# troylee/nnet-asr

Measured on AMD Instinct MI355X. Metric: training frames/sec (whole node), 440→2048×4→senone MLP, 1/2/4/8 MI355X, higher is better.
Workload: dtype f32; 1 GPU; TNet SGD step, 440x2048x2048x2048x2048x4000 sigmoid MLP + softmax xent; bunch_per_gpu=1024, global_bunch=1024, frames_resident_per_gpu=65536, parallelism=dp1

## Files before the change

### nnet-asr_amd/csrc/kernels/gemm_f32.hip

```cpp
#include <float.h>

#include <cstdlib>
#include <array>
#include <cstring>
#include <initializer_list>
#include <map>
#include <mutex>
#include <unordered_map>
#include <type_traits>

#include "kcommon.h"
#include "rbm_stats.h"
#include "gather.h"

namespace tnetk {

enum { EPI_STORE = 0, EPI_BIAS = 1, EPI_BIAS_SIG = 2, EPI_DSIG = 3, EPI_SGD = 4, EPI_BIAS_NSIG = 5,
       EPI_BIAS_NEG = 6, EPI_RBM = 7,
       EPI_DSIG_CS = 8, EPI_SGD_B = 9,
       EPI_STORE_BG = 10,
       EPI_BIAS_SIG_BIN = 11 };
constexpr int kColsumSlabRows = 32;
constexpr int kMaxSplit = 8;
constexpr int epi_base(int e) {
// ... 1585 lines not shown
              const int cl = ecol(j) + e - bn;
              if constexpr (VM == 4) {
                *reinterpret_cast<f32x4*>(ts + cl * LDP + rl0) =
                    f32x4{acc[4 * aq][NE * j + e][r], acc[4 * aq + 1][NE * j + e][r], acc[4 * aq + 2][NE * j + e][r],
                          acc[4 * aq + 3][NE * j + e][r]};
              } else {
#pragma unroll
                for (int m = 0; m < VM; ++m) ts[cl * LDP + rl0 + m] = acc[VM * aq + m][NE * j + e][r];
              }
            }
        }
      __syncthreads();
      const __amdgpu_buffer_rsrc_t rs_t = tile_rsrc(p.Ct + (long)bn * p.ldct + bm);
      for (int u = threadIdx.x; u < BN * Q; u += NT) {
        const int cl = u / Q, q4 = u % Q, col = bn + cl, row0 = bm + 4 * q4;
        if (col >= N || row0 >= M) continue;
        const f32x4 v = *reinterpret_cast<const f32x4*>(ts + cl * LDP + 4 * q4);
        if (row0 + 3 < M) {
          st_wt(rs_t, (long)cl * p.ldct + 4 * q4, v);
        } else {
#pragma unroll
          for (int m = 0; m < 4; ++m)
            if (row0 + m < M) p.Ct[(long)col * p.ldct + row0 + m] = v[m];
        }
      }
    }
  }
  }
  if constexpr (EPI == EPI_BIAS_SIG_BIN) binarize_tile<BM, BN, NT>(p, bm, bn);
  TNET_STAMP(3);
  TNET_STAMP_RT(5);
}

template <int BM, int BN, int BK, int WM, int WN, int S, bool A_KC, bool B_KC, int EPI, int SPK = 0>
__global__ __launch_bounds__(WM * WN * 64)
__attribute__((amdgpu_waves_per_eu((WM * WN + 3) / 4, (WM * WN + 3) / 4)))
void gemm16_sk_kernel(const GemmP p, const int G) {
  __shared__ __attribute__((aligned(16))) float smem[gemm16_smem_floats<BM, BN, BK, S, EPI, true>()];
  const int T = ((p.M + BM - 1) / BM) * ((p.N + BN - 1) / BN), KT = p.K / BK;
  const long I = (long)T * KT;
  const int b = blockIdx.x, xcd = b & 7, q8 = G >> 3, r8 = G & 7;
  const int v = (xcd < r8 ? xcd * (q8 + 1) : r8 * (q8 + 1) + (xcd - r8) * q8) + (b >> 3);
  const long s = (long)v * I / G, e = (long)(v + 1) * I / G;
  for (long k0 = s; k0 < e;) {
    const int t = (int)(k0 / KT);
    const long tb = (long)t * KT, te = tb + KT, k1 = e < te ? e : te;
    if (k0 != s) __syncthreads();
    const int w0 = (int)(((tb + 1) * G - 1) / I), w1 = (int)((te * G - 1) / I);
    GemmP q = p;
    q.ksplit = w1 - w0 + 1;
    const long kk = (k0 - tb) * BK;
    q.A = p.A + (A_KC ? kk : kk * p.lda);
    q.B = p.B + (B_KC ? kk : kk * p.ldb);
    q.K = (int)((k1 - k0) * BK);
    gemm16_body<BM, BN, BK, WM, WN, S, SPK, A_KC, B_KC, kEpiStreamK + EPI, true>(q, smem, t);
    k0 = k1;
  }
}

template <int BM, int BN, bool A_KC, bool B_KC, int EPI, bool PX>
__global__ __launch_bounds__(256) __attribute__((amdgpu_waves_per_eu(1, 1)))
void gemm16_split2_kernel(const GemmP p) {
  __shared__ __attribute__((aligned(16))) float smem[gemm16_smem_floats<BM, BN, 64, 2, EPI, PX>()];
  const int nwg = gridDim.x, b = blockIdx.x, xcd = b & 7, q8 = nwg >> 3, r8 = nwg & 7;
  const int v = (xcd < r8 ? xcd * (q8 + 1) : r8 * (q8 + 1) + (xcd - r8) * q8) + (b >> 3);
  GemmP q = p;
  const long kk = (long)(v & 1) * (p.K / 2);
  q.A = p.A + (A_KC ? kk : kk * p.lda);
  q.B = p.B + (B_KC ? kk : kk * p.ldb);
  q.K = p.K / 2;
  q.ksplit = 2;
  gemm16_body<BM, BN, 64, 2, 2, 2, 0, A_KC, B_KC, kEpiStreamK + EPI, PX>(q, smem, v >> 1);
}

template <int BM, int BN, int BK, int WM, int WN, int S, int SP, bool A_KC, bool B_KC, int EPI_T, bool PX = false>
__global__ __launch_bounds__((WM * WN + (SP == 2)) * 64)
__attribute__((amdgpu_waves_per_eu((WM * WN + (SP == 2) + 3) / 4, (WM * WN + (SP == 2) + 3) / 4)))
void gemm16_kernel(const GemmP p_in) {
  __shared__ __attribute__((aligned(16))) float smem[gemm16_smem_floats<BM, BN, BK, S, EPI_T, PX>()];
  gemm16_body<BM, BN, BK, WM, WN, S, SP, A_KC, B_KC, EPI_T, PX>(p_in, smem, blockIdx.x);
}

template <int BMA, int BNA, bool AKA, bool BKA, int EPIA, bool PXA, int BMB, int BNB, bool AKB, bool BKB, int EPIB,
          bool PXB, int SPA = 0, int SPB = 0, int KTA = 64, int STA = 2>
__global__ __launch_bounds__(256) __attribute__((amdgpu_waves_per_eu(1, 1)))
void gemm16_pair_kernel(const GemmP pa, const GemmP pb, const int na) {
  constexpr int SA = gemm16_smem_floats<BMA, BNA, KTA, STA, EPIA, PXA>(), SB = gemm16_smem_floats<BMB, BNB, 64, 2, EPIB, PXB>();
  __shared__ __attribute__((aligned(16))) float smem[SA > SB ? SA : SB];
  if ((int)blockIdx.x < na) gemm16_body<BMA, BNA, KTA, 2, 2, STA, SPA, AKA, BKA, EPIA, PXA>(pa, smem, blockIdx.x);
  else gemm16_body<BMB, BNB, 64, 2, 2, 2, SPB, AKB, BKB, EPIB, PXB>(pb, smem, (int)blockIdx.x - na);
}

template <int BM, int BN, int BK, int WM, int WN, int S>
__global__ __launch_bounds__(WM * WN * 64) __attribute__((amdgpu_waves_per_eu(1, 1)))
void gemm16_upd_pair_kernel(const GemmP pa, const GemmP pb, const int na) {
  __shared__ __attribute__((aligned(16))) float smem[gemm16_smem_floats<BM, BN, BK, S, EPI_SGD_B, false>()];
  if ((int)blockIdx.x < na) gemm16_body<BM, BN, BK, WM, WN, S, 0, false, false, EPI_SGD_B, false>(pa, smem, blockIdx.x);
  else gemm16_body<BM, BN, BK, WM, WN, S, 0, false, false, EPI_SGD_B, false>(pb, smem, (int)blockIdx.x - na);
}

template <int BM, int BN, int BK, int WM, int WN, int S, int EPI = EPI_SGD_B>
__global__ __launch_bounds__(WM * WN * 64) __attribute__((amdgpu_waves_per_eu(1, 1)))
void gemm16_upd_gather_kernel(const GemmP pa, const GemmP pb, const int na, const int nb, const BunchGatherP g) {
  __shared__ __attribute__((aligned(16))) float smem[gemm16_smem_floats<BM, BN, BK, S, EPI, false>()];
  const int b = blockIdx.x;
  if (b < na) gemm16_body<BM, BN, BK, WM, WN, S, 0, false, false, EPI, false>(pa, smem, b);
  else if (b < na + nb) gemm16_body<BM, BN, BK, WM, WN, S, 0, false, false, EPI, false>(pb, smem, b - na);
  else bunch_gather_block(g, b - na - nb, (int)gridDim.x - na - nb);
}

template <bool BD>
__global__ __launch_bounds__(256) __attribute__((amdgpu_waves_per_eu(1, 1)))
void gemm16_upd_mixed_gather_kernel(const GemmP pa, const GemmP pb, const int na, const int nb, const BunchGatherP g) {
  constexpr int SA = gemm16_smem_floats<128, 128, 64, 2, EPI_SGD_B, true>();
  constexpr int SB = BD ? gemm16_smem_floats<64, 64, 64, 2, EPI_SGD_B, false>()
                        : gemm16_smem_floats<64, 64, 32, 4, EPI_SGD_B, false>();
  __shared__ __attribute__((aligned(16))) float smem[SA > SB ? SA : SB];
  const int b = blockIdx.x;
  if (b < na) {
    gemm16_body<128, 128, 64, 2, 2, 2, 5, false, false, EPI_SGD_B, true>(pa, smem, b);
  } else if (b < na + nb) {
    if constexpr (BD) gemm16_body<64, 64, 64, 2, 2, 2, 5, false, false, EPI_SGD_B, false>(pb, smem, b - na);
    else gemm16_body<64, 64, 32, 4, 1, 4, 0, false, false, EPI_SGD_B, false>(pb, smem, b - na);
  } else {
    bunch_gather_block(g, b - na - nb, (int)gridDim.x - na - nb);
  }
}

template <bool PX, int SP = 0, bool BKC = true>
__global__ __launch_bounds__(256) __attribute__((amdgpu_waves_per_eu(1, 1)))
void gemm16_bwd_slabs_kernel(const GemmP p, const int na, const float* __restrict__ Et, const TnetMatrixDim dEt,
                             float* __restrict__ cpt, const long ldcpt, const int slabs, const int ncb) {
  __shared__ __attribute__((aligned(16))) float smem[gemm16_smem_floats<64, 128, 64, 2, EPI_DSIG_CS, PX>()];
  const int b = blockIdx.x;
  if (b < na) {
    gemm16_body<64, 128, 64, 2, 2, 2, SP, true, BKC, EPI_DSIG_CS, PX>(p, smem, b);
  } else {
    const int c = b - na;
    colsum_partial_block<true>(Et, dEt, cpt, slabs, 0x7fffffff, ldcpt, c % ncb, c / ncb, smem);
  }
}

__global__ __launch_bounds__(256) __attribute__((amdgpu_waves_per_eu(1, 1)))
void gemm16_rbm_update_stats_kernel(const GemmP p, const int na, const float* __restrict__ Vs, TnetMatrixDim dV,
                                    const float* __restrict__ Hs, TnetMatrixDim dH, int B, int nvb,
                                    float* __restrict__ vb, float* __restrict__ cvb, float* __restrict__ hb,
                                    float* __restrict__ chb, float scale, float mmt, double* __restrict__ stats,
                                    int nhb, const BunchGatherP g, const int ng) {
  constexpr int SG = gemm16_smem_floats<64, 64, 32, 4, EPI_RBM, false>();
  __shared__ __attribute__((aligned(16))) float smem[SG > RS_SMEM_FLOATS ? SG : RS_SMEM_FLOATS];
  const int b = blockIdx.x;
  if (b < na) gemm16_body<64, 64, 32, 4, 1, 4, 0, false, false, EPI_RBM, false>(p, smem, b);
  else if (b < na + ng) bunch_gather_block(g, b - na, ng);
  else rbm_stats_block(b - na - ng, smem, Vs, dV, Hs, dH, B, nvb, vb, cvb, hb, chb, scale, mmt, stats, nhb);
}
// ... 197 lines not shown
  X(m128x256k32s3, 1, 128, 256, 32, 2, 2, 3, 0)         \
  X(m64x64k64s2, 1, 64, 64, 64, 2, 2, 2, 0)             \
  X(m64x64k32s4, 1, 64, 64, 32, 2, 2, 4, 0)             \
  X(m32x64k64s2, 1, 32, 64, 64, 2, 2, 2, 0)             \
  X(m64x64a4, 1, 64, 64, 64, 2, 2, 2, 5)

enum GemmCfg {
#define X(name, ...) CFG_##name,
  TNET_GEMM_CFGS(X)
#undef X
  CFG_COUNT
};
static const char* kCfgNames[CFG_COUNT] = {
#define X(name, ...) #name,
    TNET_GEMM_CFGS(X)
#undef X
};

static int g_cfg = -2;
static int g_group = -1;
static int g_split = -1;
static int g_early = 1;
static int g_pair = 1;
static int g_pre0 = 1;
static int g_reserve = 0, g_cus = 0;
static int g_direct = -1;
static int g_kc = -1;
static int g_wt = 1;
extern "C" int tnetk_top_rows_shape_ok(const float* X, long ldx, const float* W, long ldw, int M, int N, int K);
extern "C" int tnetk_top_rows_partials(const float* X, long ldx, const float* W, long ldw, int M, int N, int K,
                                       float* part, long ldpart, void* stream);
static int forced_cfg();
static bool upd64_direct(const GemmP& p);
constexpr int kTopSlices = 4;
static float* splitk_workspace(size_t bytes, hipStream_t st);
static bool top_split_ok(const GemmP& p) {
  static const bool on = !(getenv("TNET_TOP_SPLIT") && getenv("TNET_TOP_SPLIT")[0] == '0');
  return on && forced_cfg() < 0 && g_split <= 0 && tnetk_top_rows_shape_ok(p.A, p.lda, p.B, p.ldb, p.M, p.N, p.K);
}
static float* top_split_partials(const GemmP& p, hipStream_t st, int* ldp_out) {
  const int ldp = 16 * ((p.N + 15) / 16);
  float* ws = splitk_workspace(sizeof(float) * kTopSlices * (size_t)p.M * ldp, st);
  if (!ws) return nullptr;
  if (tnetk_top_rows_partials(p.A, p.lda, p.B, p.ldb, p.M, p.N, p.K, ws, ldp, st) != TNET_OK) return nullptr;
  *ldp_out = ldp;
  return ws;
}
struct WeightShadow {
  float* t;
  long ld;
  int rows, cols;
  int kept;
};
static std::mutex g_shadow_mu;
static std::unordered_map<const float*, WeightShadow> g_shadow;
static thread_local int g_shadow_dropped = 0;
static void shadow_attach(GemmP& p) {
  p.Ct = nullptr;
  p.ldct = 0;
  g_shadow_dropped = 0;
  std::lock_guard<std::mutex> g(g_shadow_mu);
  auto it = g_shadow.find(p.C);
  if (it != g_shadow.end() && it->second.rows == p.M && it->second.cols == p.N) {
    p.Ct = it->second.t;
    p.ldct = it->second.ld;
  }
// ... 293 lines not shown
  int ks = 1;
  if (splittable) {
    int tbm, tbn, kind;
    cfg_shape(cfg, &tbm, &tbn, &kind);
    const long tiles = (long)cdiv(p.M, tbm) * cdiv(p.N, tbn);
    if (g_split > 0) {
      ks = g_split < kMaxSplit ? g_split : kMaxSplit;
    } else if (tiles < 100 && p.K >= 1024) {
      while (ks < kMaxSplit && tiles * ks * 2 <= 288) ks *= 2;
      const long t32 = (long)cdiv(p.M, 32) * cdiv(p.N, 64);
      if (cfg == CFG_m64x64k32s4w41 && ks >= 4 && t32 * (ks / 2) <= 288) {
        cfg = CFG_m32x64k64s2;
        kind = 1;
        ks /= 2;
      }
    }
    while (ks > 1 && (p.K % (4 * ks) != 0 || p.K / ks < 64)) ks /= 2;
    if (ks > 1 && kind != 1) cfg = CFG_m64x64k32s4w41;
  }
  return GemmPlan{cfg, ks};
}

template <bool A_KC, bool B_KC, int EPI>
static int launch_gemm(const GemmP& p_in, hipStream_t st) {
  if constexpr (EPI == EPI_DSIG_CS) {
    if constexpr (B_KC) return launch_colsum_bwd(p_in, st);
    else return launch_colsum_bwd_t(p_in, st);
  } else {
  if (p_in.M <= 0 || p_in.N <= 0) return TNET_OK;
  static const int noload = getenv("TNET_GEMM_DIAG") ? atoi(getenv("TNET_GEMM_DIAG")) : 0;
  GemmP p = p_in;
  p.diag_noload = noload;
  p.group = g_group > 0 ? g_group : 8;
  if (launch_split2<A_KC, B_KC, EPI>(p, st)) {
    TNET_LAUNCH_CHECK();
    return TNET_OK;
  }
  const GemmPlan pl = plan_gemm<A_KC>(p, epi_splittable(EPI));
  const int cfg = pl.cfg;
  if (pl.ks > 1) return launch_splitk<A_KC, B_KC, EPI>(p, cfg, pl.ks, st);
  bool sk_done = false;
  if (cfg == CFG_m64x128k64s2) sk_done = launch_sk<64, 128, A_KC, B_KC, EPI>(p, st);
  else if (cfg == CFG_m128x128k64s2) sk_done = launch_sk<128, 128, A_KC, B_KC, EPI>(p, st);
  if (sk_done) {
    TNET_LAUNCH_CHECK();
    return TNET_OK;
  }
  int rcfg = cfg;
  if (g_direct > 0 && forced_cfg() < 0 && !B_KC) {
    if (cfg == CFG_m64x128k64s2)
      rcfg = (g_direct == 3 || p.K <= 512) ? CFG_m64x128a4 : CFG_m64x128a8;
    else if (cfg == CFG_m128x128k64s2) rcfg = CFG_m128x128a4;
    else if (cfg == CFG_m128x256k32s3 && g_direct == 4) rcfg = CFG_m128x256a2;
  }
  if (g_kc >= 2 && forced_cfg() < 0 && A_KC && B_KC && cfg == CFG_m64x128k64s2) rcfg = CFG_m64x128c8;
  if constexpr (!A_KC && !B_KC && (EPI == EPI_SGD_B || EPI == EPI_SGD))
    if (forced_cfg() < 0 && cfg == CFG_m64x64k32s4w41 && upd64_direct(p)) rcfg = CFG_m64x64a4;
  bool ok = false;
  switch (rcfg) {
#define X(name, KIND, BM, BN, BK, WM, WN, S, IL) \
  case CFG_##name: ok = launch_cfg<KIND, BM, BN, BK, WM, WN, S, IL, A_KC, B_KC, EPI>(p, st); break;
    TNET_GEMM_CFGS(X)
#undef X
    default: return TNET_ERR_ARG;
  }
  if (!ok) launch_cfg<0, 64, 64, 32, 2, 2, 4, 0, A_KC, B_KC, EPI>(p, st);
// ... 84 lines not shown
static int launch_pair_upd_bwd(GemmP pu, GemmP pb, hipStream_t st) { return launch_pair_a_bwd<EPI_SGD_B>(pu, pb, st); }

static int cu_count() {
  if (!g_cus) {
    int dev = 0;
    hipDeviceProp_t prop;
    if (hipGetDevice(&dev) != hipSuccess || hipGetDeviceProperties(&prop, dev) != hipSuccess) return 0;
    g_cus = prop.multiProcessorCount;
  }
  return g_cus;
}
static bool split2_on() {
  if (g_split2 < 0) g_split2 = getenv("TNET_GEMM_SPLIT2") ? atoi(getenv("TNET_GEMM_SPLIT2")) : 0;
  return g_split2 != 0;
}

static int launch_upd_pair(GemmP pa, GemmP pb, hipStream_t st) {
  if (forced_cfg() >= 0 || !g_pair) return TNET_ERR_UNSUPPORTED;
  if (pa.M <= 0 || pa.N <= 0 || pb.M <= 0 || pb.N <= 0) return TNET_ERR_UNSUPPORTED;
  if (!g_cus) {
    int dev = 0;
    hipDeviceProp_t prop;
    if (hipGetDevice(&dev) != hipSuccess || hipGetDeviceProperties(&prop, dev) != hipSuccess)
      return TNET_ERR_UNSUPPORTED;
    g_cus = prop.multiProcessorCount;
  }
  const int na = cdiv(pa.M, 64) * cdiv(pa.N, 64), nb = cdiv(pb.M, 64) * cdiv(pb.N, 64);
  if (na + nb > g_cus - g_reserve) return TNET_ERR_UNSUPPORTED;
  for (const GemmP* q : {&pa, &pb})
    if (4 * (32L * q->lda + q->M) >= (1L << 32) || 4 * (32L * q->ldb + q->N) >= (1L << 32)) return TNET_ERR_UNSUPPORTED;
  pa.group = pb.group = g_group > 0 ? g_group : 8;
  pa.early_issue = pb.early_issue = g_early;
  pa.wt = pb.wt = g_wt;
  gemm16_upd_pair_kernel<64, 64, 32, 4, 1, 4><<<na + nb, 256, 0, st>>>(pa, pb, na);
  TNET_LAUNCH_CHECK();
  return TNET_OK;
}

static bool aligned16(const void* q) { return ((uintptr_t)q & 15) == 0; }

static int check_common(const GemmP& p) {
  if (p.M < 0 || p.N < 0 || p.K < 0) return TNET_ERR_ARG;
  if ((p.lda & 3) || (p.ldb & 3) || (p.ldc & 3)) return TNET_ERR_ARG;
  if (!aligned16(p.A) || !aligned16(p.B) || !aligned16(p.C)) return TNET_ERR_ARG;
  return TNET_OK;
}

}

using namespace tnetk;

extern "C" int tnet_sgemm(char transa, char transb, int m, int n, int k, float alpha, const float* A, int lda,
                          const float* B, int ldb, float beta, float* C, int ldc, void* stream) {
  GemmP p{};
  p.M = m; p.N = n; p.K = k;
  p.A = A; p.lda = lda; p.B = B; p.ldb = ldb; p.C = C; p.ldc = ldc;
  p.alpha = alpha; p.beta = beta;
  int st = check_common(p);
  if (st) return st;
  const bool ta = (transa == 'T' || transa == 't'), tb = (transb == 'T' || transb == 't');
  hipStream_t s = (hipStream_t)stream;
  if (k == 0) {
    if (beta == 1.f) return TNET_OK;
    TnetMatrixDim d{m, n, ldc};
    return tnetF_add_scaled(0.f, C, ldc, beta, C, d, stream);
  }
  if (!ta && !tb) return launch_gemm<true, false, EPI_STORE>(p, s);
// ... 437 lines not shown

extern "C" int tnet_affine_update_bias_pair(const float* X, TnetMatrixDim dX, const float* E, TnetMatrixDim dE,
                                           float* W, TnetMatrixDim dW, float* corrW, int strideCorr, float scale,
                                           float mmt, float l2, const float* colpart, int ldcolpart, float* b,
                                           float* corr_b, const float* X2, TnetMatrixDim dX2, const float* E2,
                                           TnetMatrixDim dE2, float* W2, TnetMatrixDim dW2, float* corrW2,
                                           int strideCorr2, float scale2, float mmt2, float l22,
                                           const float* colpart2, int ldcolpart2, float* b2, float* corr_b2,
                                           void* stream) {
  GemmP pa, pb;
  int st = update_bias_params(pa, X, dX, E, dE, W, dW, corrW, strideCorr, scale, mmt, l2, colpart, ldcolpart, b,
                              corr_b);
  if (st) return st;
  st = update_bias_params(pb, X2, dX2, E2, dE2, W2, dW2, corrW2, strideCorr2, scale2, mmt2, l22, colpart2, ldcolpart2,
                          b2, corr_b2);
  if (st) return st;
  if (W == W2 || b == b2 || (corrW && corrW == corrW2)) return TNET_ERR_ARG;
  shadow_attach(pb);
  shadow_attach(pa);
  const int rc = launch_upd_pair(pa, pb, (hipStream_t)stream);
  shadow_done(pa, rc);
  return shadow_done(pb, rc);
}

namespace tnetk {
static bool upd64_direct(const GemmP& p) {
  static const bool on = !(getenv("TNET_UPD64_DIRECT") && getenv("TNET_UPD64_DIRECT")[0] == '0');
  auto a16p = [](const void* v) { return ((uintptr_t)v & 15) == 0; };
  return on && g_direct > 0 && p.ksplit <= 1 && (long)cdiv(p.M, 64) * cdiv(p.N, 64) >= 200 && p.K / 64 >= 1 &&
         p.M % 4 == 0 && p.N % 4 == 0 && !(p.lda & 3) && !(p.ldb & 3) && a16p(p.A) && a16p(p.B) &&
         4 * ((long)p.K * p.lda) < (1L << 31) && 4 * ((long)p.K * p.ldb) < (1L << 31);
}

static bool upd_mixed_ok(const GemmP& pa, const GemmP& pb) {
  static const bool on = !(getenv("TNET_UPD_MIXED") && getenv("TNET_UPD_MIXED")[0] == '0');
  if (!on || !g_pair || g_reserve > 0 || g_direct <= 0 || forced_cfg() >= 0) return false;
  const GemmPlan la = plan_gemm<false>(pa, true), lb = plan_gemm<false>(pb, true);
  if (la.cfg != CFG_m128x128k64s2 || la.ks != 1 || lb.cfg != CFG_m64x64k32s4w41 || lb.ks != 1) return false;
  auto a16p = [](const void* v) { return ((uintptr_t)v & 15) == 0; };
  const bool dir = pa.K / 64 >= 1 && !(pa.lda & 3) && !(pa.ldb & 3) && a16p(pa.A) && a16p(pa.B) && pa.M % 4 == 0 &&
                   pa.N % 4 == 0 && 4 * ((long)pa.K * pa.lda) < (1L << 31) && 4 * ((long)pa.K * pa.ldb) < (1L << 31);
  if (!dir || !px_exact<128, 128, EPI_SGD_B>(pa)) return false;
  if (4 * (64L * pa.lda + pa.M) >= (1L << 32) || 4 * (64L * pa.ldb + pa.N) >= (1L << 32)) return false;
  if (4 * (32L * pb.lda + pb.M) >= (1L << 32) || 4 * (32L * pb.ldb + pb.N) >= (1L << 32)) return false;
  return true;
}
}

extern "C" int tnet_affine_update_bias_gather(const float* X, TnetMatrixDim dX, const float* E, TnetMatrixDim dE,
                                              float* W, TnetMatrixDim dW, float* corrW, int strideCorr, float scale,
                                              float mmt, float l2, const float* colpart, int ldcolpart, float* b,
                                              float* corr_b, const float* X2, TnetMatrixDim dX2, const float* E2,
                                              TnetMatrixDim dE2, float* W2, TnetMatrixDim dW2, float* corrW2,
                                              int strideCorr2, float scale2, float mmt2, float l22,
                                              const float* colpart2, int ldcolpart2, float* b2, float* corr_b2,
                                              float* y, const float* x, int* labels_out, const int* labels_in,
                                              const int* copy_from, TnetMatrixDim dy, TnetMatrixDim dx,
                                              void* stream) {
  GemmP pa, pb{};
  int st = update_bias_params(pa, X, dX, E, dE, W, dW, corrW, strideCorr, scale, mmt, l2, colpart, ldcolpart, b,
                              corr_b);
  if (st) return st;
  const bool two = X2 != nullptr;
  if (two) {
    st = update_bias_params(pb, X2, dX2, E2, dE2, W2, dW2, corrW2, strideCorr2, scale2, mmt2, l22, colpart2,
                            ldcolpart2, b2, corr_b2);
// ... 11 lines not shown
    return std::array<ByteSpan, 4>{span_of(q.C, q.M, q.ldc, 4), span_of(q.corr, q.M, q.ldcorr, 4),
                                   span_of(q.bvec, q.N, 1, 4), span_of(q.bcorr, q.N, 1, 4)};
  };
  shadow_attach(pa);
  if (two) shadow_attach(pb);
  const ByteSpan cta = span_of(pa.Ct, pa.N, pa.ldct, 4), ctb = span_of(two ? pb.Ct : nullptr, pb.N, pb.ldct, 4);
  const auto ra = reads(pa), rb = reads(pb);
  const auto wa = writes(pa), wb = writes(pb);
  if (!gather_independent(y, x, labels_out, labels_in, copy_from, dy, dx, {ra[0], ra[1], ra[2], rb[0], rb[1], rb[2]},
                          {wa[0], wa[1], wa[2], wa[3], wb[0], wb[1], wb[2], wb[3], cta, ctb}))
    return TNET_ERR_ARG;
  if (any_overlap({cta, ctb}, {ra[0], ra[1], ra[2], rb[0], rb[1], rb[2], wa[0], wa[1], wa[2], wa[3], wb[0], wb[1],
                               wb[2], wb[3]}) ||
      spans_overlap(cta, ctb))
    return TNET_ERR_ARG;
  const int c4 = (dy.cols + 3) & ~3;
  if (((uintptr_t)y & 15) || ((uintptr_t)x & 15) || (dy.stride & 3) || (dx.stride & 3) || c4 > dy.stride ||
      c4 > dx.stride)
    return TNET_ERR_UNSUPPORTED;
  if (forced_cfg() >= 0 || split2_on() || g_split > 0) return TNET_ERR_UNSUPPORTED;
  if (pa.M <= 0 || pa.N <= 0 || (two && (pb.M <= 0 || pb.N <= 0))) return TNET_ERR_UNSUPPORTED;
  int na, nb = 0;
  if (two && upd_mixed_ok(pa, pb)) {
    na = cdiv(pa.M, 128) * cdiv(pa.N, 128);
    nb = cdiv(pb.M, 64) * cdiv(pb.N, 64);
    const int cus = cu_count();
    if (cus <= 0) return TNET_ERR_UNSUPPORTED;
    const int spare = cus - nb;
    const int ng = spare < 8 ? 8 : spare > 64 ? 64 : spare;
    pa.group = pb.group = g_group > 0 ? g_group : 8;
    pa.early_issue = pb.early_issue = g_early;
    pa.wt = pb.wt = g_wt;
    BunchGatherP g{y, x, labels_out, labels_in, copy_from, dy.rows, c4, dy.stride, dx.stride};
    if (upd64_direct(pb)) gemm16_upd_mixed_gather_kernel<true><<<na + nb + ng, 256, 0, (hipStream_t)stream>>>(pa, pb, na, nb, g);
    else gemm16_upd_mixed_gather_kernel<false><<<na + nb + ng, 256, 0, (hipStream_t)stream>>>(pa, pb, na, nb, g);
    TNET_LAUNCH_CHECK();
    shadow_done(pa, TNET_OK);
    return shadow_done(pb, TNET_OK);
  }
  if (two) {
    if (!g_pair) return TNET_ERR_UNSUPPORTED;
    na = cdiv(pa.M, 64) * cdiv(pa.N, 64);
    nb = cdiv(pb.M, 64) * cdiv(pb.N, 64);
  } else {
    const GemmPlan pl = plan_gemm<false>(pa, epi_splittable(EPI_SGD_B));
    if (pl.cfg != CFG_m64x64k32s4w41 || pl.ks != 1) return TNET_ERR_UNSUPPORTED;
    na = cdiv(pa.M, 64) * cdiv(pa.N, 64);
  }
  for (const GemmP* q : {&pa, &pb}) {
    if (q == &pb && !two) break;
    if (4 * (32L * q->lda + q->M) >= (1L << 32) || 4 * (32L * q->ldb + q->N) >= (1L << 32)) return TNET_ERR_UNSUPPORTED;
  }
  const int cus = cu_count();
  if (cus <= 0) return TNET_ERR_UNSUPPORTED;
  const int spare = cus - g_reserve - na - nb;
  if (two && na + nb > cus - g_reserve) return TNET_ERR_UNSUPPORTED;
  if (spare < 8) return TNET_ERR_UNSUPPORTED;
  const int ng = spare < 64 ? spare : 64;
  pa.group = pb.group = g_group > 0 ? g_group : 8;
  pa.early_issue = pb.early_issue = g_early;
  pa.wt = pb.wt = g_wt;
  BunchGatherP g{y, x, labels_out, labels_in, copy_from, dy.rows, c4, dy.stride, dx.stride};
  gemm16_upd_gather_kernel<64, 64, 32, 4, 1, 4><<<na + nb + ng, 256, 0, (hipStream_t)stream>>>(pa, pb, na, nb, g);
  TNET_LAUNCH_CHECK();
  shadow_done(pa, TNET_OK);
  if (two) shadow_done(pb, TNET_OK);
  return TNET_OK;
}

static int update_bwd_pair(const float* X, TnetMatrixDim dX, const float* E, TnetMatrixDim dE, float* W,
                           TnetMatrixDim dW, float* corrW, int strideCorr, float scale, float mmt, float l2,
                           const float* colpart, int ldcolpart, float* b, float* corr_b, const float* E2,
                           TnetMatrixDim dE2, const float* W2, TnetMatrixDim dW2, const float* Ybelow, int strideYbelow,
                           float* Eo, TnetMatrixDim dEo, float* colpart2, int ldcolpart2, void* stream, bool bwd_t) {
  if (dX.rows != dE.rows || dW.rows != dX.cols || dW.cols != dE.cols || !colpart || !b || ldcolpart < dE.cols)
    return TNET_ERR_ARG;
  if (mmt != 0.f && (!corrW || !corr_b)) return TNET_ERR_ARG;
  const int w2_k = bwd_t ? dW2.rows : dW2.cols, w2_n = bwd_t ? dW2.cols : dW2.rows;
  if (dE2.cols != w2_k || dEo.rows != dE2.rows || dEo.cols != w2_n || !Ybelow || !colpart2 ||
      ldcolpart2 < dEo.cols || !aligned16(Ybelow) || (strideYbelow & 3))
    return TNET_ERR_ARG;
  if (W == W2) return TNET_ERR_ARG;
  GemmP pu{};
  pu.M = dX.cols; pu.N = dE.cols; pu.K = dX.rows;
  pu.A = X; pu.lda = dX.stride; pu.B = E; pu.ldb = dE.stride; pu.C = W; pu.ldc = dW.stride;
  pu.corr = (mmt != 0.f || corrW) ? corrW : nullptr; pu.ldcorr = strideCorr;
  if (pu.corr && (pu.ldcorr & 3)) return TNET_ERR_ARG;
  pu.scale = scale; pu.mmt = mmt; pu.l2 = l2;
  pu.bpart = colpart; pu.ldbpart = ldcolpart; pu.bslabs = tnet_colsum_slabs(dE.rows);
  pu.bvec = b; pu.bcorr = mmt != 0.f ? corr_b : nullptr; pu.bscale = scale; pu.bmmt = mmt;
  int st = check_common(pu);
  if (st) return st;
  GemmP pb{};
  pb.M = dE2.rows; pb.N = w2_n; pb.K = dE2.cols;
  pb.A = E2; pb.lda = dE2.stride; pb.B = W2; pb.ldb = dW2.stride; pb.C = Eo; pb.ldc = dEo.stride;
  pb.alpha = 1.f; pb.beta = 0.f;
// ... 136 lines not shown
                          {wa[0], wa[1], wb[0], wb[1]}))
    return TNET_ERR_ARG;
  const int c4 = (dy.cols + 3) & ~3;
  if (((uintptr_t)y & 15) || ((uintptr_t)x & 15) || (dy.stride & 3) || (dx.stride & 3) || c4 > dy.stride ||
      c4 > dx.stride)
    return TNET_ERR_UNSUPPORTED;
  if (forced_cfg() >= 0 || split2_on() || g_split > 0) return TNET_ERR_UNSUPPORTED;
  if (pa.M <= 0 || pa.N <= 0 || (two && (pb.M <= 0 || pb.N <= 0))) return TNET_ERR_UNSUPPORTED;
  int na, nb = 0;
  if (two) {
    if (!g_pair) return TNET_ERR_UNSUPPORTED;
    na = cdiv(pa.M, 64) * cdiv(pa.N, 64);
    nb = cdiv(pb.M, 64) * cdiv(pb.N, 64);
  } else {
    const GemmPlan pl = plan_gemm<false>(pa, epi_splittable(EPI_STORE_BG));
    if (pl.cfg != CFG_m64x64k32s4w41 || pl.ks != 1) return TNET_ERR_UNSUPPORTED;
    na = cdiv(pa.M, 64) * cdiv(pa.N, 64);
  }
  for (const GemmP* q : {&pa, &pb}) {
    if (q == &pb && !two) break;
    if (4 * (32L * q->lda + q->M) >= (1L << 32) || 4 * (32L * q->ldb + q->N) >= (1L << 32)) return TNET_ERR_UNSUPPORTED;
  }
  const int cus = cu_count();
  if (cus <= 0) return TNET_ERR_UNSUPPORTED;
  if (two && na + nb > cus - g_reserve) return TNET_ERR_UNSUPPORTED;
  const int spare = cus - g_reserve - na - nb;
  if (spare < 8) return TNET_ERR_UNSUPPORTED;
  const int ng = spare < 64 ? spare : 64;
  pa.group = pb.group = g_group > 0 ? g_group : 8;
  pa.early_issue = pb.early_issue = g_early;
  pa.wt = pb.wt = g_wt;
  BunchGatherP g{y, x, labels_out, labels_in, copy_from, dy.rows, c4, dy.stride, dx.stride};
  gemm16_upd_gather_kernel<64, 64, 32, 4, 1, 4, EPI_STORE_BG><<<na + nb + ng, 256, 0, (hipStream_t)stream>>>(
      pa, pb, na, nb, g);
  TNET_LAUNCH_CHECK();
  return TNET_OK;
}

extern "C" int tnet_affine_grad(const float* X, TnetMatrixDim dX, const float* E, TnetMatrixDim dE, float* G,
                                TnetMatrixDim dG, void* stream) {
  if (dX.rows != dE.rows || dG.rows != dX.cols || dG.cols != dE.cols) return TNET_ERR_ARG;
  GemmP p{};
  p.M = dX.cols; p.N = dE.cols; p.K = dX.rows;
  p.A = X; p.lda = dX.stride; p.B = E; p.ldb = dE.stride; p.C = G; p.ldc = dG.stride;
  p.alpha = 1.f; p.beta = 0.f;
  int st = check_common(p);
  if (st) return st;
  return launch_gemm<false, false, EPI_STORE>(p, (hipStream_t)stream);
}

extern "C" int tnet_gemm_config(const char* name) {
  forced_cfg();
  char base[64] = "auto";
  int split = -1, rsv = -1, s2 = -1;
  if (name) {
    const char* plus = strchr(name, '+');
    const size_t n = plus ? (size_t)(plus - name) : strlen(name);
    if (n >= sizeof(base)) return TNET_ERR_ARG;
    memcpy(base, name, n);
    base[n] = 0;
    while (plus) {
      if (!strncmp(plus, "+sk", 3) && atoi(plus + 3) >= 1) split = atoi(plus + 3);
      else if (!strncmp(plus, "+rsv", 4) && plus[4] >= '0' && plus[4] <= '9') rsv = atoi(plus + 4);
      else if (!strncmp(plus, "+s2", 3) && (plus[3] == '0' || plus[3] == '1')) s2 = plus[3] - '0';
      else return TNET_ERR_ARG;
      plus = strchr(plus + 1, '+');
    }
  }
  int cfg = -2;
  if (!strcmp(base, "auto")) cfg = -1;
  for (int i = 0; i < CFG_COUNT; i++)
    if (!strcmp(base, kCfgNames[i])) cfg = i;
  if (cfg == -2) return TNET_ERR_ARG;
  g_cfg = cfg;
  g_split = split;
  if (rsv >= 0) g_reserve = rsv;
  if (s2 >= 0) g_split2 = s2;
  return TNET_OK;
}

extern "C" int tnet_gemm_reserve(int cus) {
  if (cus < 0) return TNET_ERR_ARG;
  forced_cfg();
  g_reserve = cus;
  return TNET_OK;
}

#ifdef TNET_GEMM_STAMP
extern "C" int tnet_diag_stamps(unsigned long long* host, int n_wg) {
  if (n_wg > 8192) n_wg = 8192;
  return hipMemcpyFromSymbol(host, HIP_SYMBOL(g_tnet_stamps), sizeof(unsigned long long) * 6 * n_wg, 0,
                             hipMemcpyDeviceToHost) == hipSuccess ? TNET_OK : TNET_ERR_LAUNCH;
}
extern "C" int tnet_diag_stamps_clear() {
  void* a = nullptr;
  if (hipGetSymbolAddress(&a, HIP_SYMBOL(g_tnet_stamps)) != hipSuccess) return TNET_ERR_RUNTIME;
  return hipMemset(a, 0, sizeof(g_tnet_stamps)) == hipSuccess && hipDeviceSynchronize() == hipSuccess
             ? TNET_OK : TNET_ERR_RUNTIME;
}
#endif
```

Measured before the change: 1.019 million frames/s.

## Add intra-block K-split 64x64 weight-update kernel with register-ring buffer loads

Adds a new 64x64 SGD weight-update GEMM body in which each of the four waves takes a quarter of the K range. Each wave streams its operands directly from global memory into a register ring using buffer loads interleaved with MFMAs, and the partial tiles are reduced through LDS before the fused SGD/momentum/bias epilogue. It is dispatched automatically wherever the planner would pick the 64x64 direct-update config, including the pair, gather and mixed-gather launchers. The aim is to avoid LDS staging and the per-K-step barriers on the tall-K update GEMMs. In exchange it uses a large register footprint and adds a cross-wave reduction step.

```diff
diff --git a/nnet-asr_amd/csrc/kernels/gemm_f32.hip b/nnet-asr_amd/csrc/kernels/gemm_f32.hip
--- a/nnet-asr_amd/csrc/kernels/gemm_f32.hip
+++ b/nnet-asr_amd/csrc/kernels/gemm_f32.hip
@@ -1641,6 +1641,212 @@
   TNET_STAMP_RT(5);
 }
 
+constexpr int kKsplitSmemFloats = 3 * 64 * 64;
+template <int EPI>
+__device__ __forceinline__ void upd64_ksplit_body(const GemmP& p, float* __restrict__ smem, const int bid_x) {
+  static_assert(EPI == EPI_SGD || EPI == EPI_SGD_B, "SGD epilogues only");
+  constexpr int BM = 64, BN = 64, DD = 4, NR = 8;
+  TNET_STAMP_RT(4);
+  TNET_STAMP(0);
+  const int M = p.M, N = p.N, K = p.K;
+  const int nbn = (N + BN - 1) / BN, nbm = (M + BM - 1) / BM;
+  const int nwg = nbm * nbn;
+  const int bid = bid_x, xcd = bid & 7, q8 = nwg >> 3, r8 = nwg & 7;
+  const int L = (xcd < r8 ? xcd * (q8 + 1) : r8 * (q8 + 1) + (xcd - r8) * q8) + (bid >> 3);
+  const int grp = p.group, per_group = grp * nbn;
+  const int first_m = (L / per_group) * grp;
+  const int gsz = min(nbm - first_m, grp);
+  const int bm = (first_m + (L % per_group) % gsz) * BM, bn = ((L % per_group) / gsz) * BN;
+
+  const int lane = threadIdx.x & 63, wid = __builtin_amdgcn_readfirstlane(threadIdx.x >> 6);
+  const int lg = lane >> 4, li = lane & 15;
+  const int KQ = 16 * ((((K + 3) >> 2) + 15) >> 4);
+  const int k0 = wid * KQ, k1 = min(K, k0 + KQ);
+  const int nch = (k1 - k0) >> 4, rem = (k1 - k0) & 15;
+
+  const int ca = max(min(bm + 4 * li, M - 4), 0), cb = max(min(bn + 4 * li, N - 4), 0);
+  unsigned oA[4], oB[4];
+#pragma unroll
+  for (int s = 0; s < 4; ++s) {
+    oA[s] = 4u * (unsigned)((4 * lg + s) * p.lda + ca);
+    oB[s] = 4u * (unsigned)((4 * lg + s) * p.ldb + cb);
+  }
+  const int cA = 64 * p.lda, cB = 64 * p.ldb;
+  const unsigned long long ba = (unsigned long long)(uintptr_t)(p.A + (long)k0 * p.lda),
+                           bb = (unsigned long long)(uintptr_t)(p.B + (long)k0 * p.ldb);
+  const u32x4 dA = {(unsigned)ba, (unsigned)(ba >> 32), 0x7FFFFFF0u, 0x00020000u};
+  const u32x4 dB = {(unsigned)bb, (unsigned)(bb >> 32), 0x7FFFFFF0u, 0x00020000u};
+
+  f32x4 acc[4][4];
+#pragma unroll
+  for (int a = 0; a < 4; ++a)
+#pragma unroll
+    for (int b = 0; b < 4; ++b) acc[a][b] = f32x4{0.f, 0.f, 0.f, 0.f};
+
+  f32x4 ring[DD][NR];
+  auto ld = [&](int c, int r) {
+    f32x4 v;
+    if (r < 4) asm volatile("buffer_load_dwordx4 %0, %1, %2, %3 offen" : "=v"(v) : "v"(oA[r]), "s"(dA), "s"(c * cA));
+    else asm volatile("buffer_load_dwordx4 %0, %1, %2, %3 offen" : "=v"(v) : "v"(oB[r - 4]), "s"(dB), "s"(c * cB));
+    return v;
+  };
+  constexpr int WV = (DD - 2) * NR;
+  auto wait_slot = [&](f32x4 (&q)[NR]) {
+    asm volatile("s_waitcnt vmcnt(%8)"
+                 : "+v"(q[0]), "+v"(q[1]), "+v"(q[2]), "+v"(q[3]), "+v"(q[4]), "+v"(q[5]), "+v"(q[6]), "+v"(q[7])
+                 : "n"(WV));
+  };
+#pragma unroll
+  for (int j = 0; j < DD - 1; ++j)
+#pragma unroll
+    for (int r = 0; r < NR; ++r) ring[j][r] = ld(min(j, nch - 1), r);
+  asm volatile("" ::: "memory");
+
+  const int erow0 = bm + 16 * lg + 4 * wid, ecol = bn + 4 * li;
+  const bool has_q = p.corr != nullptr;
+  f32x4 pre_w[4], pre_q[4];
+#pragma unroll
+  for (int a = 0; a < 4; ++a) {
+    pre_w[a] = pre_q[a] = f32x4{0.f, 0.f, 0.f, 0.f};
+    if (erow0 + a < M && ecol < N) {
+      pre_w[a] = *reinterpret_cast<const f32x4*>(p.C + (long)(erow0 + a) * p.ldc + ecol);
+      if (has_q) pre_q[a] = *reinterpret_cast<const f32x4*>(p.corr + (long)(erow0 + a) * p.ldcorr + ecol);
+    }
+  }
+  BiasPre bpre;
+  if constexpr (EPI == EPI_SGD_B)
+    if (bm == 0) bias_pre_load<BN, false>(p, bn, bpre);
+  TNET_STAMP(1);
+
+  auto chunk_mfmas = [&](const f32x4 (&q)[NR], auto&& filler) {
+    int mi = 0;
+#pragma unroll
+    for (int s2 = 0; s2 < 4; ++s2)
+#pragma unroll
+      for (int a = 0; a < 4; ++a)
+#pragma unroll
+        for (int b = 0; b < 4; ++b) {
+          acc[a][b] = __builtin_amdgcn_mfma_f32_16x16x4f32(q[s2][a], q[4 + s2][b], acc[a][b], 0, 0, 0);
+          filler(mi);
+          ++mi;
+        }
+  };
+  for (int c0 = 0; c0 < nch; c0 += DD) {
+#pragma unroll
+    for (int j = 0; j < DD; ++j) {
+      if (c0 + j >= nch) break;
+      const int cn = min(c0 + j + DD - 1, nch - 1);
+      __builtin_amdgcn_sched_barrier(0);
+      wait_slot(ring[j]);
+      __builtin_amdgcn_sched_barrier(0);
+      chunk_mfmas(ring[j], [&](int mi) {
+        if (mi < NR) {
+          __builtin_amdgcn_sched_barrier(0);
+          ring[(j + DD - 1) % DD][mi] = ld(cn, mi);
+          __builtin_amdgcn_sched_barrier(0);
+        }
+      });
+    }
+  }
+  asm volatile("s_waitcnt vmcnt(0)" ::: "memory");
+  if (rem) {
+    f32x4 t[NR];
+#pragma unroll
+    for (int s = 0; s < 4; ++s) {
+      const int k = k0 + 16 * nch + 4 * lg + s, kk = min(k, K - 1);
+      const f32x4 x = *reinterpret_cast<const f32x4*>(p.A + (long)kk * p.lda + ca);
+      const f32x4 e = *reinterpret_cast<const f32x4*>(p.B + (long)kk * p.ldb + cb);
+      const f32x4 z = {0.f, 0.f, 0.f, 0.f};
+      t[s] = k < k1 ? x : z;
+      t[4 + s] = k < k1 ? e : z;
+    }
+    chunk_mfmas(t, [](int) {});
+  }
+  TNET_STAMP(2);
+
+  auto vec = [&](int a, int r) { return f32x4{acc[a][0][r], acc[a][1][r], acc[a][2][r], acc[a][3][r]}; };
+  f32x4 own[4];
+#pragma unroll
+  for (int r = 0; r < 4; ++r) {
+    if (wid == r) {
+#pragma unroll
+      for (int a = 0; a < 4; ++a) own[a] = vec(a, r);
+    } else {
+      const int sl = wid < r ? wid : wid - 1;
+#pragma unroll
+      for (int a = 0; a < 4; ++a)
+        *reinterpret_cast<f32x4*>(smem + ((4 * r + a) * 3 + sl) * 256 + 4 * lane) = vec(a, r);
+    }
+  }
+  __syncthreads();
+  const __amdgpu_buffer_rsrc_t rs_c = tile_rsrc(p.C + (long)bm * p.ldc + bn);
+  const __amdgpu_buffer_rsrc_t rs_q = tile_rsrc(p.corr ? p.corr + (long)bm * p.ldcorr + bn : p.C);
+  f32x4 part[4][3];
+#pragma unroll
+  for (int a = 0; a < 4; ++a)
+#pragma unroll
+    for (int sl = 0; sl < 3; ++sl)
+      part[a][sl] = *reinterpret_cast<const f32x4*>(smem + ((4 * wid + a) * 3 + sl) * 256 + 4 * lane);
+  f32x4 upd[4];
+#pragma unroll
+  for (int a = 0; a < 4; ++a) upd[a] = f32x4{0.f, 0.f, 0.f, 0.f};
+#pragma unroll
+  for (int a = 0; a < 4; ++a) {
+    const int row = erow0 + a;
+    if (row >= M || ecol >= N) continue;
+    const f32x4 p0 = wid == 0 ? own[a] : part[a][0];
+    const f32x4 p1 = wid == 0 ? part[a][0] : wid == 1 ? own[a] : part[a][1];
+    const f32x4 p2 = wid <= 1 ? part[a][1] : wid == 2 ? own[a] : part[a][2];
+    const f32x4 p3 = wid == 3 ? own[a] : part[a][2];
+    const f32x4 v = ((p0 + p1) + p2) + p3;
+    f32x4 o, qn;
+#pragma unroll
+    for (int e = 0; e < 4; ++e) {
+      const float c = has_q ? v[e] + p.mmt * pre_q[a][e] : v[e];
+      qn[e] = c;
+      float w = pre_w[a][e];
+      w = w + p.scale * c;
+      w = w + p.l2 * w;
+      o[e] = w;
+    }
+    upd[a] = o;
+    if (p.wt) {
+      st_wt(rs_c, (long)(row - bm) * p.ldc + (ecol - bn), o);
+      if (has_q) st_wt(rs_q, (long)(row - bm) * p.ldcorr + (ecol - bn), qn);
+    } else {
+      *reinterpret_cast<f32x4*>(p.C + (long)row * p.ldc + ecol) = o;
+      if (has_q) *reinterpret_cast<f32x4*>(p.corr + (long)row * p.ldcorr + ecol) = qn;
+    }
+  }
+  if (p.Ct) {
+    constexpr int LDP = BM + 4, Q = BM / 4;
+    static_assert(BN * LDP <= kKsplitSmemFloats, "shadow image fits the partial tiles' LDS");
+    __syncthreads();
+#pragma unroll
+    for (int e = 0; e < 4; ++e)
+      *reinterpret_cast<f32x4*>(smem + (4 * li + e) * LDP + 16 * lg + 4 * wid) =
+          f32x4{upd[0][e], upd[1][e], upd[2][e], upd[3][e]};
+    __syncthreads();
+    const __amdgpu_buffer_rsrc_t rs_t = tile_rsrc(p.Ct + (long)bn * p.ldct + bm);
+    for (int u = threadIdx.x; u < BN * Q; u += 256) {
+      const int cl = u / Q, q4 = u % Q;
+      if (bn + cl >= N || bm + 4 * q4 >= M) continue;
+      st_wt(rs_t, (long)cl * p.ldct + 4 * q4, *reinterpret_cast<const f32x4*>(smem + cl * LDP + 4 * q4));
+    }
+  }
+  if constexpr (EPI == EPI_SGD_B)
+    if (bm == 0) bias_pre_finish<BN, false>(p, bn, bpre);
+  TNET_STAMP(3);
+  TNET_STAMP_RT(5);
+}
+
+template <int EPI>
+__global__ __launch_bounds__(256) __attribute__((amdgpu_waves_per_eu(1, 1)))
+void gemm16_upd_ksplit_kernel(const GemmP p) {
+  __shared__ __attribute__((aligned(16))) float smem[kKsplitSmemFloats];
+  upd64_ksplit_body<EPI>(p, smem, blockIdx.x);
+}
+
 template <int BM, int BN, int BK, int WM, int WN, int S, bool A_KC, bool B_KC, int EPI, int SPK = 0>
 __global__ __launch_bounds__(WM * WN * 64)
 __attribute__((amdgpu_waves_per_eu((WM * WN + 3) / 4, (WM * WN + 3) / 4)))
@@ -1700,36 +1906,55 @@
   else gemm16_body<BMB, BNB, 64, 2, 2, 2, SPB, AKB, BKB, EPIB, PXB>(pb, smem, (int)blockIdx.x - na);
 }
 
-template <int BM, int BN, int BK, int WM, int WN, int S>
+template <int BM, int BN, int BK, int WM, int WN, int S, bool KS = false>
 __global__ __launch_bounds__(WM * WN * 64) __attribute__((amdgpu_waves_per_eu(1, 1)))
-void gemm16_upd_pair_kernel(const GemmP pa, const GemmP pb, const int na) {
+void gemm16_upd_pair_kernel(const GemmP pa, const GemmP pb, const int na, const int ksa, const int ksb) {
+  static_assert(!KS || (BM == 64 && BN == 64 && WM * WN == 4 && S * (BM + BN) * BK >= kKsplitSmemFloats), "ksplit tile");
   __shared__ __attribute__((aligned(16))) float smem[gemm16_smem_floats<BM, BN, BK, S, EPI_SGD_B, false>()];
-  if ((int)blockIdx.x < na) gemm16_body<BM, BN, BK, WM, WN, S, 0, false, false, EPI_SGD_B, false>(pa, smem, blockIdx.x);
-  else gemm16_body<BM, BN, BK, WM, WN, S, 0, false, false, EPI_SGD_B, false>(pb, smem, (int)blockIdx.x - na);
-}
-
-template <int BM, int BN, int BK, int WM, int WN, int S, int EPI = EPI_SGD_B>
+  const int b = blockIdx.x;
+  if constexpr (KS) {
+    if (b < na ? ksa : ksb) {
+      upd64_ksplit_body<EPI_SGD_B>(b < na ? pa : pb, smem, b < na ? b : b - na);
+      return;
+    }
+  }
+  if (b < na) gemm16_body<BM, BN, BK, WM, WN, S, 0, false, false, EPI_SGD_B, false>(pa, smem, b);
+  else gemm16_body<BM, BN, BK, WM, WN, S, 0, false, false, EPI_SGD_B, false>(pb, smem, b - na);
+}
+
+template <int BM, int BN, int BK, int WM, int WN, int S, int EPI = EPI_SGD_B, bool KS = false>
 __global__ __launch_bounds__(WM * WN * 64) __attribute__((amdgpu_waves_per_eu(1, 1)))
-void gemm16_upd_gather_kernel(const GemmP pa, const GemmP pb, const int na, const int nb, const BunchGatherP g) {
+void gemm16_upd_gather_kernel(const GemmP pa, const GemmP pb, const int na, const int nb, const BunchGatherP g,
+                              const int ksa, const int ksb) {
+  static_assert(!KS || (EPI == EPI_SGD_B && BM == 64 && BN == 64 && WM * WN == 4 &&
+                        S * (BM + BN) * BK >= kKsplitSmemFloats), "ksplit tile");
   __shared__ __attribute__((aligned(16))) float smem[gemm16_smem_floats<BM, BN, BK, S, EPI, false>()];
   const int b = blockIdx.x;
+  if constexpr (KS) {
+    if (b < na + nb && (b < na ? ksa : ksb)) {
+      upd64_ksplit_body<EPI_SGD_B>(b < na ? pa : pb, smem, b < na ? b : b - na);
+      return;
+    }
+  }
   if (b < na) gemm16_body<BM, BN, BK, WM, WN, S, 0, false, false, EPI, false>(pa, smem, b);
   else if (b < na + nb) gemm16_body<BM, BN, BK, WM, WN, S, 0, false, false, EPI, false>(pb, smem, b - na);
   else bunch_gather_block(g, b - na - nb, (int)gridDim.x - na - nb);
 }
 
-template <bool BD>
+template <int BD>
 __global__ __launch_bounds__(256) __attribute__((amdgpu_waves_per_eu(1, 1)))
 void gemm16_upd_mixed_gather_kernel(const GemmP pa, const GemmP pb, const int na, const int nb, const BunchGatherP g) {
   constexpr int SA = gemm16_smem_floats<128, 128, 64, 2, EPI_SGD_B, true>();
-  constexpr int SB = BD ? gemm16_smem_floats<64, 64, 64, 2, EPI_SGD_B, false>()
+  constexpr int SB = BD == 2 ? kKsplitSmemFloats
+                   : BD ? gemm16_smem_floats<64, 64, 64, 2, EPI_SGD_B, false>()
                         : gemm16_smem_floats<64, 64, 32, 4, EPI_SGD_B, false>();
   __shared__ __attribute__((aligned(16))) float smem[SA > SB ? SA : SB];
   const int b = blockIdx.x;
   if (b < na) {
     gemm16_body<128, 128, 64, 2, 2, 2, 5, false, false, EPI_SGD_B, true>(pa, smem, b);
   } else if (b < na + nb) {
-    if constexpr (BD) gemm16_body<64, 64, 64, 2, 2, 2, 5, false, false, EPI_SGD_B, false>(pb, smem, b - na);
+    if constexpr (BD == 2) upd64_ksplit_body<EPI_SGD_B>(pb, smem, b - na);
+    else if constexpr (BD == 1) gemm16_body<64, 64, 64, 2, 2, 2, 5, false, false, EPI_SGD_B, false>(pb, smem, b - na);
     else gemm16_body<64, 64, 32, 4, 1, 4, 0, false, false, EPI_SGD_B, false>(pb, smem, b - na);
   } else {
     bunch_gather_block(g, b - na - nb, (int)gridDim.x - na - nb);
@@ -1993,6 +2218,8 @@
                                        float* part, long ldpart, void* stream);
 static int forced_cfg();
 static bool upd64_direct(const GemmP& p);
+static int g_ks = 0;
+static bool upd64_ksplit(const GemmP& p);
 constexpr int kTopSlices = 4;
 static float* splitk_workspace(size_t bytes, hipStream_t st);
 static bool top_split_ok(const GemmP& p) {
@@ -2352,6 +2579,14 @@
   GemmP p = p_in;
   p.diag_noload = noload;
   p.group = g_group > 0 ? g_group : 8;
+  if constexpr (!A_KC && !B_KC && (EPI == EPI_SGD_B || EPI == EPI_SGD)) {
+    if (upd64_ksplit(p)) {
+      p.wt = g_wt;
+      gemm16_upd_ksplit_kernel<EPI><<<cdiv(p.M, 64) * cdiv(p.N, 64), 256, 0, st>>>(p);
+      TNET_LAUNCH_CHECK();
+      return TNET_OK;
+    }
+  }
   if (launch_split2<A_KC, B_KC, EPI>(p, st)) {
     TNET_LAUNCH_CHECK();
     return TNET_OK;
@@ -2502,7 +2737,9 @@
   pa.group = pb.group = g_group > 0 ? g_group : 8;
   pa.early_issue = pb.early_issue = g_early;
   pa.wt = pb.wt = g_wt;
-  gemm16_upd_pair_kernel<64, 64, 32, 4, 1, 4><<<na + nb, 256, 0, st>>>(pa, pb, na);
+  const int ksa = upd64_ksplit(pa), ksb = upd64_ksplit(pb);
+  if (ksa || ksb) gemm16_upd_pair_kernel<64, 64, 32, 4, 1, 4, true><<<na + nb, 256, 0, st>>>(pa, pb, na, ksa, ksb);
+  else gemm16_upd_pair_kernel<64, 64, 32, 4, 1, 4><<<na + nb, 256, 0, st>>>(pa, pb, na, 0, 0);
   TNET_LAUNCH_CHECK();
   return TNET_OK;
 }
@@ -3006,6 +3243,21 @@
          4 * ((long)p.K * p.lda) < (1L << 31) && 4 * ((long)p.K * p.ldb) < (1L << 31);
 }
 
+static bool upd64_ksplit_covers(const GemmP& p) {
+  auto a16p = [](const void* v) { return ((uintptr_t)v & 15) == 0; };
+  return p.ksplit <= 1 && p.K >= 256 && p.M > 0 && p.N > 0 && p.M % 4 == 0 && p.N % 4 == 0 && !(p.lda & 3) &&
+         !(p.ldb & 3) && !(p.ldc & 3) && a16p(p.A) && a16p(p.B) && a16p(p.C) &&
+         (!p.Ct || 4 * (64L * p.ldct) < (1L << 31)) &&
+         (!p.corr || (a16p(p.corr) && !(p.ldcorr & 3) && 4 * (64L * p.ldcorr) < (1L << 31))) &&
+         4 * ((long)p.K * p.lda) < (1L << 31) && 4 * ((long)p.K * p.ldb) < (1L << 31) && 4 * (64L * p.ldc) < (1L << 31);
+}
+static bool upd64_ksplit(const GemmP& p) {
+  if (forced_cfg() >= 0 || !upd64_ksplit_covers(p)) return false;
+  if (g_ks > 0) return true;
+  const GemmPlan pl = plan_gemm<false>(p, true);
+  return pl.cfg == CFG_m64x64k32s4w41 && pl.ks == 1 && upd64_direct(p);
+}
+
 static bool upd_mixed_ok(const GemmP& pa, const GemmP& pb) {
   static const bool on = !(getenv("TNET_UPD_MIXED") && getenv("TNET_UPD_MIXED")[0] == '0');
   if (!on || !g_pair || g_reserve > 0 || g_direct <= 0 || forced_cfg() >= 0) return false;
@@ -3083,8 +3335,9 @@
     pa.early_issue = pb.early_issue = g_early;
     pa.wt = pb.wt = g_wt;
     BunchGatherP g{y, x, labels_out, labels_in, copy_from, dy.rows, c4, dy.stride, dx.stride};
-    if (upd64_direct(pb)) gemm16_upd_mixed_gather_kernel<true><<<na + nb + ng, 256, 0, (hipStream_t)stream>>>(pa, pb, na, nb, g);
-    else gemm16_upd_mixed_gather_kernel<false><<<na + nb + ng, 256, 0, (hipStream_t)stream>>>(pa, pb, na, nb, g);
+    if (upd64_ksplit(pb)) gemm16_upd_mixed_gather_kernel<2><<<na + nb + ng, 256, 0, (hipStream_t)stream>>>(pa, pb, na, nb, g);
+    else if (upd64_direct(pb)) gemm16_upd_mixed_gather_kernel<1><<<na + nb + ng, 256, 0, (hipStream_t)stream>>>(pa, pb, na, nb, g);
+    else gemm16_upd_mixed_gather_kernel<0><<<na + nb + ng, 256, 0, (hipStream_t)stream>>>(pa, pb, na, nb, g);
     TNET_LAUNCH_CHECK();
     shadow_done(pa, TNET_OK);
     return shadow_done(pb, TNET_OK);
@@ -3112,7 +3365,12 @@
   pa.early_issue = pb.early_issue = g_early;
   pa.wt = pb.wt = g_wt;
   BunchGatherP g{y, x, labels_out, labels_in, copy_from, dy.rows, c4, dy.stride, dx.stride};
-  gemm16_upd_gather_kernel<64, 64, 32, 4, 1, 4><<<na + nb + ng, 256, 0, (hipStream_t)stream>>>(pa, pb, na, nb, g);
+  const int ksa = upd64_ksplit(pa), ksb = two && upd64_ksplit(pb);
+  if (ksa || ksb)
+    gemm16_upd_gather_kernel<64, 64, 32, 4, 1, 4, EPI_SGD_B, true><<<na + nb + ng, 256, 0, (hipStream_t)stream>>>(
+        pa, pb, na, nb, g, ksa, ksb);
+  else
+    gemm16_upd_gather_kernel<64, 64, 32, 4, 1, 4><<<na + nb + ng, 256, 0, (hipStream_t)stream>>>(pa, pb, na, nb, g, 0, 0);
   TNET_LAUNCH_CHECK();
   shadow_done(pa, TNET_OK);
   if (two) shadow_done(pb, TNET_OK);
@@ -3315,7 +3573,7 @@
   pa.wt = pb.wt = g_wt;
   BunchGatherP g{y, x, labels_out, labels_in, copy_from, dy.rows, c4, dy.stride, dx.stride};
   gemm16_upd_gather_kernel<64, 64, 32, 4, 1, 4, EPI_STORE_BG><<<na + nb + ng, 256, 0, (hipStream_t)stream>>>(
-      pa, pb, na, nb, g);
+      pa, pb, na, nb, g, 0, 0);
   TNET_LAUNCH_CHECK();
   return TNET_OK;
 }
@@ -3335,7 +3593,7 @@
 extern "C" int tnet_gemm_config(const char* name) {
   forced_cfg();
   char base[64] = "auto";
-  int split = -1, rsv = -1, s2 = -1;
+  int split = -1, rsv = -1, s2 = -1, ks = -1;
   if (name) {
     const char* plus = strchr(name, '+');
     const size_t n = plus ? (size_t)(plus - name) : strlen(name);
@@ -3344,6 +3602,7 @@
     base[n] = 0;
     while (plus) {
       if (!strncmp(plus, "+sk", 3) && atoi(plus + 3) >= 1) split = atoi(plus + 3);
+      else if (!strncmp(plus, "+ks", 3) && (plus[3] == '0' || plus[3] == '1')) ks = plus[3] - '0';
       else if (!strncmp(plus, "+rsv", 4) && plus[4] >= '0' && plus[4] <= '9') rsv = atoi(plus + 4);
       else if (!strncmp(plus, "+s2", 3) && (plus[3] == '0' || plus[3] == '1')) s2 = plus[3] - '0';
       else return TNET_ERR_ARG;
@@ -3359,6 +3618,7 @@
   g_split = split;
   if (rsv >= 0) g_reserve = rsv;
   if (s2 >= 0) g_split2 = s2;
+  if (ks >= 0) g_ks = ks;
   return TNET_OK;
 }
 
```

Result: no change. 1.022 million frames/s (median of 6 runs) (+0.3%).
